# YuvalNirkin/hyperseg

Hardware: AMD Instinct MI355X
Metric: frames/sec @ bs=1 HyperSeg-M 1024x512 (higher is better)
Workload: dtype f32 storage and accumulation; level-4 inverted residual products as 3-term f16 splits (f32-class: 1.3e-7 of sum|a||b|; exact_f32 beside it)

## Files before the change

hyperseg_amd/_hip.py:

```python
import ctypes as C
import os

import torch

_LIB_PATH = os.environ.get('HS_HIP_LIB') or os.path.join(os.path.dirname(os.path.abspath(__file__)), 'lib',
                                                         'libhyperseg_hip.so')

ACT_NONE, ACT_RELU, ACT_RELU6, ACT_SWISH = 0, 1, 2, 3
PAD_MODES = {'zeros': 0, 'reflect': 1, 'replicate': 2, 'circular': 3}
PREV_NONE, PREV_SAME, PREV_BILINEAR = 0, 1, 2

_STATUS = {-1: 'bad argument', -2: 'feature map does not tile into the weight grid (H % fh or W % fw != 0)',
           -3: 'unsupported shape', -4: 'tile does not fit the LDS'}


class HipLibraryError(RuntimeError):
    pass


class StageInputC(C.Structure):
    _fields_ = [('skip', C.c_void_p), ('prev', C.c_void_p),
                ('batch', C.c_int32), ('H', C.c_int32), ('W', C.c_int32),
                ('c_skip', C.c_int32), ('c_prev', C.c_int32),
                ('Hp', C.c_int32), ('Wp', C.c_int32),
# ... 112 lines not shown
        'hs_patch_conv_plain_fwd': ([i32, vp, vp, i64, i32, i32, i32, i32, i32, i32, i32, i32, i32, i32, i32, vp, vp], C.c_int),
        'hs_patch_conv_plain_bwd_in': ([i32, vp, vp, i64, i32, i32, i32, i32, i32, i32, i32, i32, i32, i32, i32, vp, vp], C.c_int),
        'hs_patch_conv_plain_bwd_w': ([i32, vp, vp, i32, i32, i32, i32, i32, i32, i32, i32, i32, i32, i32, vp, i64, vp], C.c_int),
        'hs_depthwise_conv_fwd': ([vp, i32, i32, i32, i32, vp, i32, i32, i32, i32, i32, i32, vp, vp, i32, vp, vp, vp, vp, vp], C.c_int),
        'hs_pointwise_conv_fwd': ([vp, i32, i32, i32, vp, i32, vp, vp, vp, i32, vp, vp, vp], C.c_int),
        'hs_affine_act_fwd': ([vp, i32, i32, i32, vp, vp, i32, vp, vp, vp], C.c_int),
        'hs_patch_conv_bn_fwd': ([i32, vp, vp, vp, vp, vp, vp, C.c_float, C.c_float, i32, vp, vp, vp, vp, i64, i32, i32, i32, i32, i32, i32, i32, vp, vp], C.c_int),
        'hs_patch_conv_bn_bwd_w': ([i32, vp, vp, vp, vp, vp, vp, i32, i32, i32, i32, i32, i32, i32, i32, vp, i64, vp], C.c_int),
        'hs_bootstrap_mean_of_batch_fwd': ([vp, i32, i32, i32, C.c_float, vp, vp, vp, vp], C.c_int),
        'hs_bootstrap_mean_of_batch_bwd': ([vp, i32, i32, vp, vp, vp, vp], C.c_int),
        'hs_adam_blocks': ([vp, i32], C.c_int64),
        'hs_adam_step': ([vp, vp, vp, vp, vp, i32, vp, C.c_float, C.c_double, C.c_double, C.c_float, C.c_float, i32, i32, vp, vp], C.c_int),
        'hs_adam_step_amp': ([vp, vp, vp, vp, vp, i32, vp, C.c_float, C.c_double, C.c_double, C.c_float, C.c_float, i32, i32, vp, vp, vp, vp], C.c_int),
        'hs_depthwise_pool_blocks': ([i32, i32], C.c_int),
        'hs_depthwise_conv_se_fwd': ([vp, i32, i32, i32, i32, vp, i32, i32, i32, i32, i32, i32, vp, vp, i32, vp, vp, vp, C.POINTER(SeTailC), vp], C.c_int),
        'hs_mbconv_expand_dw_se_fwd': ([vp, i32, i32, i32, i32, vp, i32, vp, vp, vp, i32, i32, i32, i32, i32, i32, vp, vp, vp, C.POINTER(SeTailC), vp], C.c_int),
        'hs_se_tail_workspace': ([i32, i32, i32, i32, i64], C.c_int64),
        'hs_se_tail_tails': ([i32, i32, i32, i64], C.c_int),
        'hs_mbconv_se_workgroups': ([i32, i32, i32, i32, i32, i32], C.c_int64),
        'hs_stem_conv_fwd': ([vp, i32, i32, i32, i32, vp, i32, i32, i32, i32, i32, vp, vp, vp, vp], C.c_int),
        'hs_mbconv_tiles': ([i32, i32, i32, i32], C.c_int),
        'hs_stem_dw_fwd': ([vp, i32, i32, i32, vp, i32, vp, vp, i32, i32, i32, i32, vp, i32, i32, i32, vp, vp, vp, vp, vp], C.c_int),
        'hs_mbconv_expand_dw_fwd': ([vp, i32, i32, i32, i32, vp, i32, vp, vp, vp, i32, i32, i32, i32, i32, i32, vp, vp, vp, vp, vp], C.c_int),
        'hs_se_gate_fwd': ([vp, i32, i32, i32, C.c_float, vp, vp, i32, vp, vp, vp, vp, vp, i32, vp, vp, vp], C.c_int),
        'hs_gemm_split_kp': ([i32], C.c_int),
        'hs_gemm_split_fwd': ([vp, vp, vp, vp, vp, i32, vp, vp, i32, i32, i32, i32, i32, vp], C.c_int),
        'hs_gemm_split_conv2x2_fwd': ([vp, vp, vp, vp, i32, vp, vp, i32, i32, i32, i32, i32, i32, vp], C.c_int),
        'hs_gemm_split_up2_fwd': ([vp, vp, vp, vp, i32, vp, i32, i32, i32, i32, i32, i32, vp], C.c_int),
        'hs_pooled_shift_fwd': ([vp, i32, C.c_float, vp, vp, vp, i32, i32, vp], C.c_int),
    }
    for name, (argtypes, restype) in sig.items():
        fn = getattr(lib, name)
        fn.argtypes, fn.restype = argtypes, restype
    if lib.hs_version() != 1:
        raise HipLibraryError(f'ABI mismatch: library reports version {lib.hs_version()}, binding expects 1')
    return lib


lib = _load()
EXPORTS = ['hs_version', 'hs_build_info', 'hs_signal2weights_fwd', 'hs_signal2weights_multi_fwd', 'hs_s2w_pack_floats', 'hs_s2w_pack_fwd', 'hs_bank_pack_fwd', 'hs_bn_fold_fwd',
           'hs_patch_conv_fwd', 'hs_patch_conv_s2w_fwd', 'hs_k1_chain_workspace', 'hs_k1_chain_fwd', 'hs_decoder_chain_workspace', 'hs_decoder_chain_fwd', 'hs_meta_conv_fwd', 'hs_meta_conv_bwd', 'hs_patch_conv_gen_fwd', 'hs_patch_ir_fwd', 'hs_patch_ir_v0_fwd', 'hs_patch_ir_v0_ws_fwd', 'hs_patch_ir_v0_workspace', 'hs_patch_ir_route', 'hs_ir_tile_map', 'hs_upsample_bilinear_fwd', 'hs_upsample_argmax_fwd',
           'hs_stage_input_fwd', 'hs_depthwise_conv_fwd', 'hs_depthwise_pool_blocks', 'hs_stem_conv_fwd', 'hs_stem_dw_fwd', 'hs_mbconv_tiles', 'hs_mbconv_expand_dw_fwd', 'hs_se_gate_fwd', 'hs_depthwise_conv_se_fwd', 'hs_mbconv_expand_dw_se_fwd', 'hs_se_tail_workspace', 'hs_se_tail_tails', 'hs_mbconv_se_workgroups', 'hs_pointwise_conv_fwd', 'hs_affine_act_fwd', 'hs_gemm_split_kp', 'hs_gemm_split_fwd', 'hs_gemm_split_conv2x2_fwd', 'hs_gemm_split_up2_fwd', 'hs_pooled_shift_fwd', 'hs_patch_conv_bwd_input',
           'hs_patch_conv_bwd_weight', 'hs_halo_tiles_fwd', 'hs_halo_tiles_bwd', 'hs_tile_interior_fwd', 'hs_tile_interior_bwd', 'hs_dw_tiles_fwd', 'hs_dw_tiles_bwd_in', 'hs_dw_tiles_bwd_w',
           'hs_s2w_train_fwd', 'hs_s2w_train_workspace', 'hs_s2w_train_bwd', 'hs_cross_entropy_fwd', 'hs_cross_entropy_bwd', 'hs_cross_entropy_typed_fwd', 'hs_cross_entropy_typed_bwd', 'hs_bootstrapped_ce_fwd', 'hs_bootstrapped_ce_bwd', 'hs_bootstrap_mean_workspace', 'hs_bootstrap_mean_fwd', 'hs_bootstrap_mean_bwd', 'hs_bootstrap_mean_batched_fwd', 'hs_bootstrap_mean_batched_bwd', 'hs_bn_train_workspace', 'hs_bn_train_stats_fwd', 'hs_dw_tiles_bn_fwd', 'hs_dw_tiles_bn_bwd_w', 'hs_patch_conv_bn_fwd', 'hs_patch_conv_bn_bwd_w', 'hs_adam_blocks', 'hs_adam_step', 'hs_bootstrap_mean_of_batch_fwd', 'hs_bootstrap_mean_of_batch_bwd', 'hs_upsample_bilinear_bwd', 'hs_upsample_bilinear_typed_bwd', 'hs_upsample_bilinear_bf16_fwd', 'hs_stage_input_typed_fwd', 'hs_bank_unpack_fwd', 'hs_bn_act_train_fwd',
           'hs_bn_act_train_bwd', 'hs_dw_tiles_bn_bwd_in_partials', 'hs_dw_tiles_bn_bwd_in', 'hs_bn_act_train_bwd_apply', 'hs_patch_conv_plain_fwd', 'hs_patch_conv_plain_bwd_in', 'hs_patch_conv_plain_bwd_w',
           'hs_upsample_bilinear_f16_fwd', 'hs_adam_step_amp']


def check(status, what):
    if status == 0:
        return
    if status < 0:
        raise HipLibraryError(f'{what}: {_STATUS.get(status, status)}')
    raise HipLibraryError(f'{what}: HIP launch failed with hipError_t {status}')


def dev_ptr(t, name='tensor', dtype=torch.float32):
    if t is None:
        return None
    if not isinstance(t, torch.Tensor):
        raise TypeError(f'{name} must be a torch.Tensor')
    if not t.is_cuda:
        raise HipLibraryError(f'{name} is on {t.device}: the HyperSeg decoder path runs on an MI355X only '
                              '(hyperseg_amd has no CPU fallback)')
    if t.dtype != dtype:
# ... 26 lines not shown
```

hyperseg_amd/build.py:

```python
import os
import shutil
import subprocess
import sys

PKG = os.path.dirname(os.path.abspath(__file__))
REPO = os.path.dirname(PKG)
CSRC = os.path.join(PKG, 'csrc')
LIB_DIR = os.path.join(PKG, 'lib')
LIB_PATH = os.path.join(LIB_DIR, 'libhyperseg_hip.so')
SOURCES = ['hs_weights.hip', 'hs_patch_conv.hip', 'hs_patch_conv_gen.hip', 'hs_patch_conv_k1m.hip', 'hs_k1_chain.hip', 'hs_meta_conv.hip', 'hs_patch_ir.hip', 'hs_patch_ir_fused.hip', 'hs_patch_irc.hip', 'hs_patch_ir_px.hip', 'hs_patch_ir_d2.hip', 'hs_encoder.hip', 'hs_mbconv.hip', 'hs_mbconv_lean.hip', 'hs_gemm_split.hip', 'hs_patch_conv_bwd.hip', 'hs_patch_conv_train.hip', 'hs_train_aux.hip', 'hs_s2w_train.hip']
HEADERS = [os.path.join(CSRC, 'hs_common.h'), os.path.join(CSRC, 'hs_ir_tiles.h'), os.path.join(CSRC, 'hs_ir_common.h'), os.path.join(CSRC, 'hs_s2w_blocked.h'), os.path.join(CSRC, 'hs_se_tail.h'), os.path.join(REPO, 'include', 'hyperseg_hip.h')]
FLAGS = ['--offload-arch=gfx950', '-O3', '-std=c++17', '-fPIC', '-ffp-contract=off', '-mllvm', '-amdgpu-kernarg-preload-count=16',
         '-Wall', '-Wno-unused-function', '-I', os.path.join(REPO, 'include'), '-I', CSRC]


def _hipcc():
    for cand in (os.environ.get('HIPCC'), shutil.which('hipcc'), '/opt/rocm/bin/hipcc'):
        if cand and os.path.exists(cand):
            return cand
    raise RuntimeError('hipcc not found (need ROCm >= 7.0 with gfx950 support)')


def needs_build():
    if not os.path.exists(LIB_PATH):
        return True
    t = os.path.getmtime(LIB_PATH)
    deps = [os.path.join(CSRC, s) for s in SOURCES] + HEADERS + [os.path.abspath(__file__)]
    return any(os.path.getmtime(d) > t for d in deps)


def build(force=False, verbose=False, extra_flags=(), sources=None, lib_path=None, obj_suffix=''):
    if sources is None and lib_path is None and not force and not needs_build():
        return LIB_PATH
    sources = list(sources or SOURCES)
# ... 28 lines not shown
```

hyperseg_amd/csrc/hs_gemm_split.hip:

```cpp
#include "hs_common.h"
#include <type_traits>

namespace hs {

using half8 = __attribute__((ext_vector_type(8))) _Float16;
using gs_f32x4 = __attribute__((ext_vector_type(4))) float;

__device__ __forceinline__ int gs_exp_of(float m) { return min(max(__float_as_int(m) >> 23, 27), 254); }
__device__ __forceinline__ float gs_scale_of(int eb) { return __int_as_float((268 - eb) << 23); }
__device__ __forceinline__ float gs_inv_scale_of(int eb) { return __int_as_float((eb - 14) << 23); }

struct GemmSplitArgs {
    const _Float16* __restrict__ wf;
    const float* __restrict__ w_inv;
    const float* __restrict__ gate; const float* __restrict__ x;
    const float* shift;
    const float* residual;
    float* y;
    int M, K, KST, N, act;
    int conv_wo;
    float* pool_partial;
    int up2_wo;
};

#ifndef HS_GS_NARROW_MAX_WG
#define HS_GS_NARROW_MAX_WG 128
#endif

#ifndef HS_GS_TALL_MIN_WG
#define HS_GS_TALL_MIN_WG 257
#endif

template <int KS, int NWV, bool FAST, int NS, int MT, int NCH, bool PATCH>
// ... 114 lines not shown
#pragma unroll
                for (int j = 0; j < 8; ++j) {
                    const float mk = (FAST || PATCH ? k0 : k0 + j) < a.K ? 1.0f : 0.0f;
                    float g = mk;
                    if constexpr (!PATCH) g = gb ? gv[c][s][j] * mk : mk;
                    xv[c][t][s][j] *= g;
                    mx = max(mx, __float_as_uint(xv[c][t][s][j]) & 0x7fffffffu);
                }
            }
            {
                auto r16 = __builtin_amdgcn_permlane16_swap(mx, mx, false, false);
                mx = max(r16[0], r16[1]);
                auto r32 = __builtin_amdgcn_permlane32_swap(mx, mx, false, false);
                mx = max(r32[0], r32[1]);
            }
            const int eb = gs_exp_of(__uint_as_float(mx));
            const float sc = gs_scale_of(eb);
            invb[t] = gs_inv_scale_of(eb);
#pragma unroll
            for (int s = 0; s < KS; ++s) {
                if constexpr (FAST || PATCH) {
                    unsigned hh[4], ll[4];
#pragma unroll
                    for (int j = 0; j < 4; ++j) {
                        asm("v_fma_mixlo_f16 %0, %2, %4, 0\n\t"
                            "v_fma_mixhi_f16 %0, %3, %4, 0\n\t"
                            "v_fma_mixlo_f16 %1, %2, %4, -%0 op_sel_hi:[0,0,1]\n\t"
                            "v_fma_mixhi_f16 %1, %3, %4, -%0 op_sel:[0,0,1] op_sel_hi:[0,0,1]"
                            : "=&v"(hh[j]), "=&v"(ll[j]) : "v"(xv[c][t][s][2 * j]), "v"(xv[c][t][s][2 * j + 1]), "v"(sc));
                    }
                    using gs_u32x4 = __attribute__((ext_vector_type(4))) unsigned;
                    bh[t][s] = __builtin_bit_cast(half8, gs_u32x4{hh[0], hh[1], hh[2], hh[3]});
                    bl[t][s] = __builtin_bit_cast(half8, gs_u32x4{ll[0], ll[1], ll[2], ll[3]});
                } else {
#pragma unroll
                    for (int j = 0; j < 8; ++j) {
                        const float v = xv[c][t][s][j] * sc;
                        const _Float16 hi = (_Float16)v;
                        bh[t][s][j] = hi;
                        bl[t][s][j] = (_Float16)(v - (float)hi);
                    }
                }
            }
        }
        if (c == 0) {
            load_a(1);
            if constexpr (LATE_TAIL) load_tail();
        }
        __builtin_amdgcn_sched_barrier(0);
#pragma unroll
        for (int mt = 0; mt < MT; ++mt) {
            const int q = c * MT + mt;
            gs_f32x4 acc[NS];
#pragma unroll
// ... 207 lines not shown
```

hyperseg_amd/functional.py:

```python
import ctypes as C
import functools
import os
import threading

import torch

from . import _hip
from ._hip import ACT_NONE, ACT_RELU, ACT_RELU6, PAD_MODES

BN_EPS_DEFAULT = 1e-5
S2W_TRAIN_MAX_LAYERS = 8
USE_SIDE_STREAM = os.environ.get('HS_SIDE_STREAM', '0') == '1'
PIPELINE_BANKS = os.environ.get('HS_SIDE_STREAM', '0') == '2'
COSCHEDULE_BANKS = os.environ.get('HS_COSCHEDULE_BANKS', '0') == '1'


def _round_up(n, m):
    return (n + m - 1) // m * m


def _device_of(a):
    if isinstance(a, torch.Tensor):
        return a.device
    if isinstance(a, (StageInput, BankRef, SignalRef)):
# ... 830 lines not shown
            d, gate, _ws = desc
            st = _hip.lib.hs_mbconv_expand_dw_se_fwd(_hip.dev_ptr(x, 'x'), b, cin, h, w, _hip.dev_ptr(w_expand, 'w_expand'), cmid,
                                                     _hip.dev_ptr(scale0, 'scale0'), _hip.dev_ptr(shift0, 'shift0'),
                                                     _hip.dev_ptr(w_dw, 'w_dw'), k, stride, pad_top, pad_left, ho, wo,
                                                     _hip.dev_ptr(scale1, 'scale1'), _hip.dev_ptr(shift1, 'shift1'), y.data_ptr(),
                                                     C.byref(d), _hip.stream_ptr())
            _hip.check(st, 'hs_mbconv_expand_dw_se_fwd')
            return y, gate, True
    partial = None
    if pool:
        partial = torch.empty(b * cmid, _hip.lib.hs_mbconv_tiles(k, stride, ho, wo), device=x.device, dtype=torch.float32)
    st = _hip.lib.hs_mbconv_expand_dw_fwd(_hip.dev_ptr(x, 'x'), b, cin, h, w, _hip.dev_ptr(w_expand, 'w_expand'), cmid,
                                          _hip.dev_ptr(scale0, 'scale0'), _hip.dev_ptr(shift0, 'shift0'),
                                          _hip.dev_ptr(w_dw, 'w_dw'), k, stride, pad_top, pad_left, ho, wo,
                                          _hip.dev_ptr(scale1, 'scale1'), _hip.dev_ptr(shift1, 'shift1'), y.data_ptr(),
                                          partial.data_ptr() if pool else None, _hip.stream_ptr())
    _hip.check(st, 'hs_mbconv_expand_dw_fwd')
    if se is not None and pool:
        return y, partial, False
    return (y, partial) if pool else y


@_on_operand_device
def pointwise_conv(x, weight, gate=None, scale=None, shift=None, act=0, residual=None):
    b, cin, h, w = x.shape
    cout = weight.shape[0]
    y = torch.empty(b, cout, h, w, device=x.device, dtype=torch.float32)
    opt = lambda t, n: _hip.dev_ptr(t, n) if t is not None else None
    st = _hip.lib.hs_pointwise_conv_fwd(_hip.dev_ptr(x, 'x'), b, cin, h * w, _hip.dev_ptr(weight, 'weight'), cout,
                                        opt(gate, 'gate'), opt(scale, 'scale'), opt(shift, 'shift'), int(act),
                                        opt(residual, 'residual'), y.data_ptr(), _hip.stream_ptr())
    _hip.check(st, 'hs_pointwise_conv_fwd')
    return y


@_on_operand_device
def affine_act_(x, scale, shift, act=0, residual=None):
    b, c, h, w = x.shape
    st = _hip.lib.hs_affine_act_fwd(_hip.dev_ptr(x, 'x'), b, c, h * w,
                                    _hip.dev_ptr(scale, 'scale') if scale is not None else None,
                                    _hip.dev_ptr(shift, 'shift'), int(act),
                                    _hip.dev_ptr(residual, 'residual') if residual is not None else None, x.data_ptr(),
                                    _hip.stream_ptr())
    _hip.check(st, 'hs_affine_act_fwd')
    return x

# ... 216 lines not shown
```

hyperseg_amd/utils/inference.py:

```python
import contextlib
import os

import torch
import torch.nn as nn


@torch.no_grad()
def _fold(conv, bn):
    scale = bn.weight / torch.sqrt(bn.running_var + bn.eps)
    shift = bn.bias - bn.running_mean * scale
    conv.weight.mul_(scale.view(-1, 1, 1, 1))
    if conv.bias is not None:
        conv.bias.mul_(scale).add_(shift)
    else:
        conv.bias = nn.Parameter(shift.clone())


def _fold_pairs(module, pairs):
    n = 0
    for conv_name, bn_name in pairs:
        conv, bn = getattr(module, conv_name, None), getattr(module, bn_name, None)
        if isinstance(conv, nn.Conv2d) and isinstance(bn, nn.BatchNorm2d) and not bn.training:
            _fold(conv, bn)
            setattr(module, bn_name, nn.Identity())
# ... 3 lines not shown

def _fold_sequential(seq):
    n = 0
    mods = list(seq)
    for i in range(len(mods) - 1):
        if isinstance(mods[i], nn.Conv2d) and isinstance(mods[i + 1], nn.BatchNorm2d) and not mods[i + 1].training:
            _fold(mods[i], mods[i + 1])
            seq[i + 1] = nn.Identity()
            n += 1
    return n


def _bn_affine(bn):
    with torch.no_grad():
        scale = bn.weight / torch.sqrt(bn.running_var + bn.eps)
        shift = bn.bias - bn.running_mean * scale
    return scale.detach().clone(), shift.detach().clone()


SPLIT_GEMM_MAX_K = int(os.environ.get('HS_SPLIT_GEMM_MAX_K', '1280'))
STEM_DW = os.environ.get('HS_STEM_DW', '1') != '0'
FUSE_EXPAND_MIN_PIXELS = int(os.environ.get('HS_FUSE_EXPAND_MIN_PIXELS', '2048'))
FUSE_EXPAND_MAX_CIN = int(os.environ.get('HS_FUSE_EXPAND_MAX_CIN', '40'))


LEAN_MFMA_MAX_CIN = int(os.environ.get('HS_LEAN_MFMA_MAX_CIN', '16'))
PW_MFMA_MAX_CIN = int(os.environ.get('HS_PW_MFMA_MAX_CIN', '96'))
PW_MFMA_MIN_PIXELS = int(os.environ.get('HS_PW_MFMA_MIN_PIXELS', '8192'))
GEMM_LT_MIN_PIXELS = int(os.environ.get('HS_GEMM_LT_MIN_PIXELS', '16384'))


@contextlib.contextmanager
def gemm_library(pixels, batch=1):
    want = os.environ.get('HS_BLAS') or ('cublaslt' if (pixels >= GEMM_LT_MIN_PIXELS or batch > 1) else 'cublas')
    prev = torch.backends.cuda.preferred_blas_library()
    torch.backends.cuda.preferred_blas_library(want)
    try:
        yield
    finally:
        torch.backends.cuda.preferred_blas_library(prev)


class FusedPointwise(nn.Module):

    def __init__(self, conv, bn, act=0):
        super().__init__()
# ... 111 lines not shown
            self.pad_w, self.pad_h = conv._pad[0] + conv._pad[1], conv._pad[2] + conv._pad[3]
        else:
            self.pad_t, self.pad_l = conv.padding
            self.pad_h, self.pad_w = 2 * conv.padding[0], 2 * conv.padding[1]
        self.skip = blk.stride == 1 and blk.in_f == blk.out_f
        self._exp_t = None
        self._red_w = None
        self.se_tail = True
        self._stem = None
        if in_offset is not None:
            assert self.expand is not None, 'a depthwise conv cannot consume an offset tensor (zero padding)'
            self.expand.absorb_input_offset(in_offset)
        with torch.no_grad():
            carried = self.project.shift.clone()
            if self.skip and in_offset is not None:
                carried += in_offset.to(carried.device)
            self.defer_shift = bool(defer_shift)
            self.out_offset = carried.clone() if defer_shift else None
            self.project.shift.copy_(torch.zeros_like(carried) if defer_shift else carried)

    def fuses_expand(self, x, ho, wo):
        return self.expand is not None and x.shape[1] <= FUSE_EXPAND_MAX_CIN and ho * wo >= FUSE_EXPAND_MIN_PIXELS

    def forward(self, inputs, blk):
        from .. import functional as HF
        pre = None
        if self._stem is not None and inputs.shape[1] == 3:
            stem = self._stem[0]
            img = inputs.contiguous()
            pre = HF.stem_dw(img, stem.w28, stem.scale, stem.shift, stem.pad_t, stem.pad_l, stem.out_size(img),
                             blk._depthwise_conv.weight, self.pad_t, self.pad_l, self.scale, self.shift, pool=True) if STEM_DW else None
            inputs = pre[0] if pre is not None else stem(img)
        x = inputs.contiguous()
        b, _, h, w = x.shape
        ho = (h + self.pad_h - self.k) // self.stride + 1
        wo = (w + self.pad_w - self.k) // self.stride + 1
        lean = True
        red, exp = blk._se_reduce, blk._se_expand
        if self._exp_t is None or self._exp_t.device != x.device:
            self._exp_t = exp.weight.detach().flatten(1).t().contiguous()
        if self._red_w is None or self._red_w.device != x.device:
            self._red_w = red.weight.detach().flatten(1)
        proj = self.project
        cmid = blk._depthwise_conv.weight.shape[0]
        lean_gemm = lean and (cmid > LEAN_MFMA_MAX_CIN if self.defer_shift else not proj.mfma_covers(cmid, ho * wo))
        folds = lean_gemm and not (proj.split_gemm and proj.split_weights(True, x.device) is not None)
        se = (self._red_w, red.bias, self._exp_t, exp.bias) if self.se_tail and not folds else None
        if pre is not None:
            out = (pre[0], pre[1], False) if se is not None else pre
        elif self.fuses_expand(x, ho, wo):
            out = HF.mbconv_expand_dw(x, self.expand.conv.weight, self.expand.scale, self.expand.shift,
                                      blk._depthwise_conv.weight, self.stride, self.pad_t, self.pad_l, (ho, wo),
                                      self.scale, self.shift, pool=True, se=se)
        else:
            in_scale = in_shift = None
            if self.expand is not None:
                if lean and not self.expand.uses_mfma(x):
                    in_scale, in_shift = self.expand.scale, self.expand.shift
                    x = self.expand.raw(x)
                else:
                    x = self.expand(x)
            out = HF.depthwise_conv_bn_act(x, blk._depthwise_conv.weight, self.stride, self.pad_t, self.pad_l,
                                           (ho, wo), self.scale, self.shift, act=3, pool=True,
                                           in_scale=in_scale, in_shift=in_shift, se=se)
        y, pooled, gated = out if se is not None else (out[0], out[1], False)

        def se_gate(**fold):
            if gated and not fold:
                return pooled
            return HF.se_gate(pooled, b, ho * wo, red.weight, red.bias, self._exp_t, exp.bias, **fold)
        skip = inputs.contiguous() if self.skip else None
        if lean_gemm:
            sw = proj.split_weights(True, y.device) if proj.split_gemm else None
            if sw is not None:
                gate = se_gate()
                if self.defer_shift:
# ... 319 lines not shown
```

include/hyperseg_hip.h:

```cpp
#ifndef HYPERSEG_HIP_H
#define HYPERSEG_HIP_H

#include <stdint.h>

#ifdef __cplusplus
extern "C" {
#endif

#define HS_ABI_VERSION 1

typedef enum {
    HS_OK = 0,
    HS_ERR_BAD_ARG = -1,
    HS_ERR_NOT_DIVISIBLE = -2,
    HS_ERR_UNSUPPORTED = -3,
    HS_ERR_LDS = -4
} hs_status;

typedef enum { HS_ACT_NONE = 0, HS_ACT_RELU = 1, HS_ACT_RELU6 = 2, HS_ACT_SWISH = 3 } hs_act;
typedef enum { HS_PAD_ZEROS = 0, HS_PAD_REFLECT = 1, HS_PAD_REPLICATE = 2, HS_PAD_CIRCULAR = 3 } hs_pad_mode;
typedef enum { HS_PREV_NONE = 0, HS_PREV_SAME = 1, HS_PREV_BILINEAR = 2 } hs_prev_mode;

typedef struct {
    const float* skip;
// ... 158 lines not shown
                             const float* w, int32_t k, int32_t stride, int32_t pad_t, int32_t pad_l,
                             int32_t Ho, int32_t Wo, const float* scale, const float* shift, int32_t act,
                             float* y, const float* in_scale, const float* in_shift, const hs_se_tail* se, void* stream);
int hs_se_gate_fwd(const float* partial, int32_t batch, int32_t channels, int32_t nblk, float inv_hw,
                   const float* w_reduce, const float* b_reduce, int32_t c_squeezed, const float* w_expand,
                   const float* b_expand, float* squeezed, float* gate, const float* w_proj, int32_t c_out,
                   const float* out_scale, float* w_scaled, void* stream);


int hs_stem_conv_fwd(const float* x, int32_t batch, int32_t c_in, int32_t H, int32_t W, const float* w, int32_t c_out,
                     int32_t pad_t, int32_t pad_l, int32_t Ho, int32_t Wo, const float* scale, const float* shift,
                     float* y, void* stream);

int hs_mbconv_tiles(int32_t k, int32_t stride, int32_t Ho, int32_t Wo);
int hs_stem_dw_fwd(const float* x, int32_t batch, int32_t H, int32_t W, const float* w_stem28, int32_t c_mid,
                   const float* scale0, const float* shift0, int32_t stem_pad_t, int32_t stem_pad_l, int32_t Hs, int32_t Ws,
                   const float* w_dw, int32_t k, int32_t pad_t, int32_t pad_l, const float* scale1, const float* shift1,
                   float* y, float* pool_partial, void* stream);
int hs_mbconv_expand_dw_fwd(const float* x, int32_t batch, int32_t c_in, int32_t H, int32_t W,
                            const float* w_expand, int32_t c_mid, const float* scale0, const float* shift0,
                            const float* w_dw, int32_t k, int32_t stride, int32_t pad_t, int32_t pad_l,
                            int32_t Ho, int32_t Wo, const float* scale1, const float* shift1, float* y,
                            float* pool_partial, void* stream);
int64_t hs_mbconv_se_workgroups(int32_t batch, int32_t c_mid, int32_t k, int32_t stride, int32_t Ho, int32_t Wo);
int hs_mbconv_expand_dw_se_fwd(const float* x, int32_t batch, int32_t c_in, int32_t H, int32_t W,
                               const float* w_expand, int32_t c_mid, const float* scale0, const float* shift0,
                               const float* w_dw, int32_t k, int32_t stride, int32_t pad_t, int32_t pad_l,
                               int32_t Ho, int32_t Wo, const float* scale1, const float* shift1, float* y,
                               const hs_se_tail* se, void* stream);

int hs_pointwise_conv_fwd(const float* x, int32_t batch, int32_t c_in, int32_t pixels, const float* w, int32_t c_out,
                          const float* gate, const float* scale, const float* shift, int32_t act, const float* residual,
                          float* y, void* stream);

int hs_affine_act_fwd(const float* x, int32_t batch, int32_t channels, int32_t pixels, const float* scale,
                      const float* shift, int32_t act, const float* residual, float* y, void* stream);

int hs_gemm_split_kp(int32_t c_in);
int hs_gemm_split_fwd(const void* w_frag, const float* w_inv, const float* gate, const float* x, const float* shift,
                      int32_t act, const float* residual, float* y, int32_t batch, int32_t c_out, int32_t c_in, int32_t kp,
                      int32_t pixels, void* stream);
int hs_gemm_split_conv2x2_fwd(const void* w_frag, const float* w_inv, const float* x, const float* shift, int32_t act, float* y,
                              float* pool_partial, int32_t batch, int32_t c_out, int32_t c_in, int32_t kp, int32_t Ho,
                              int32_t Wo, void* stream);
int hs_gemm_split_up2_fwd(const void* w_frag, const float* w_inv, const float* x, const float* shift, int32_t act, float* y,
                          int32_t batch, int32_t c_out, int32_t c_in, int32_t kp, int32_t Ho, int32_t Wo, void* stream);
// ... 112 lines not shown
```

Baseline: 1354.

## Fuse split-f16 MFMA expand conv with depthwise conv for late MBConv blocks

Adds a kernel for later MBConv blocks (wider inputs, up to 96 channels) that runs the 1x1 expand conv as a 3-term f16-split MFMA GEMM straight into an LDS band tile. It then applies BN+swish, runs the depthwise conv with BN+swish from LDS, and writes per-band pool partials for SE. This avoids writing and reading back the expanded activation in global memory and saves a launch. In exchange, each workgroup recomputes halo rows, LDS use limits occupancy, and only certain shape instantiations are supported; other shapes fall back to the old path.

```diff
diff --git a/hyperseg_amd/_hip.py b/hyperseg_amd/_hip.py
--- a/hyperseg_amd/_hip.py
+++ b/hyperseg_amd/_hip.py
@@ -158,6 +158,8 @@
         'hs_mbconv_tiles': ([i32, i32, i32, i32], C.c_int),
         'hs_stem_dw_fwd': ([vp, i32, i32, i32, vp, i32, vp, vp, i32, i32, i32, i32, vp, i32, i32, i32, vp, vp, vp, vp, vp], C.c_int),
         'hs_mbconv_expand_dw_fwd': ([vp, i32, i32, i32, i32, vp, i32, vp, vp, vp, i32, i32, i32, i32, i32, i32, vp, vp, vp, vp, vp], C.c_int),
+        'hs_mbconv_late_pool_blocks': ([i32, i32, i32, i32, i32, i32, i32, i32, i32, i32, i32], C.c_int),
+        'hs_mbconv_late_fwd': ([vp, i32, i32, i32, i32, vp, vp, i32, i32, vp, vp, vp, i32, i32, i32, i32, i32, i32, vp, vp, vp, vp, i32, i32, vp], C.c_int),
         'hs_se_gate_fwd': ([vp, i32, i32, i32, C.c_float, vp, vp, i32, vp, vp, vp, vp, vp, i32, vp, vp, vp], C.c_int),
         'hs_gemm_split_kp': ([i32], C.c_int),
         'hs_gemm_split_fwd': ([vp, vp, vp, vp, vp, i32, vp, vp, i32, i32, i32, i32, i32, vp], C.c_int),
@@ -176,7 +178,7 @@
 lib = _load()
 EXPORTS = ['hs_version', 'hs_build_info', 'hs_signal2weights_fwd', 'hs_signal2weights_multi_fwd', 'hs_s2w_pack_floats', 'hs_s2w_pack_fwd', 'hs_bank_pack_fwd', 'hs_bn_fold_fwd',
            'hs_patch_conv_fwd', 'hs_patch_conv_s2w_fwd', 'hs_k1_chain_workspace', 'hs_k1_chain_fwd', 'hs_decoder_chain_workspace', 'hs_decoder_chain_fwd', 'hs_meta_conv_fwd', 'hs_meta_conv_bwd', 'hs_patch_conv_gen_fwd', 'hs_patch_ir_fwd', 'hs_patch_ir_v0_fwd', 'hs_patch_ir_v0_ws_fwd', 'hs_patch_ir_v0_workspace', 'hs_patch_ir_route', 'hs_ir_tile_map', 'hs_upsample_bilinear_fwd', 'hs_upsample_argmax_fwd',
-           'hs_stage_input_fwd', 'hs_depthwise_conv_fwd', 'hs_depthwise_pool_blocks', 'hs_stem_conv_fwd', 'hs_stem_dw_fwd', 'hs_mbconv_tiles', 'hs_mbconv_expand_dw_fwd', 'hs_se_gate_fwd', 'hs_depthwise_conv_se_fwd', 'hs_mbconv_expand_dw_se_fwd', 'hs_se_tail_workspace', 'hs_se_tail_tails', 'hs_mbconv_se_workgroups', 'hs_pointwise_conv_fwd', 'hs_affine_act_fwd', 'hs_gemm_split_kp', 'hs_gemm_split_fwd', 'hs_gemm_split_conv2x2_fwd', 'hs_gemm_split_up2_fwd', 'hs_pooled_shift_fwd', 'hs_patch_conv_bwd_input',
+           'hs_stage_input_fwd', 'hs_depthwise_conv_fwd', 'hs_depthwise_pool_blocks', 'hs_stem_conv_fwd', 'hs_stem_dw_fwd', 'hs_mbconv_tiles', 'hs_mbconv_expand_dw_fwd', 'hs_mbconv_late_pool_blocks', 'hs_mbconv_late_fwd', 'hs_se_gate_fwd', 'hs_depthwise_conv_se_fwd', 'hs_mbconv_expand_dw_se_fwd', 'hs_se_tail_workspace', 'hs_se_tail_tails', 'hs_mbconv_se_workgroups', 'hs_pointwise_conv_fwd', 'hs_affine_act_fwd', 'hs_gemm_split_kp', 'hs_gemm_split_fwd', 'hs_gemm_split_conv2x2_fwd', 'hs_gemm_split_up2_fwd', 'hs_pooled_shift_fwd', 'hs_patch_conv_bwd_input',
            'hs_patch_conv_bwd_weight', 'hs_halo_tiles_fwd', 'hs_halo_tiles_bwd', 'hs_tile_interior_fwd', 'hs_tile_interior_bwd', 'hs_dw_tiles_fwd', 'hs_dw_tiles_bwd_in', 'hs_dw_tiles_bwd_w',
            'hs_s2w_train_fwd', 'hs_s2w_train_workspace', 'hs_s2w_train_bwd', 'hs_cross_entropy_fwd', 'hs_cross_entropy_bwd', 'hs_cross_entropy_typed_fwd', 'hs_cross_entropy_typed_bwd', 'hs_bootstrapped_ce_fwd', 'hs_bootstrapped_ce_bwd', 'hs_bootstrap_mean_workspace', 'hs_bootstrap_mean_fwd', 'hs_bootstrap_mean_bwd', 'hs_bootstrap_mean_batched_fwd', 'hs_bootstrap_mean_batched_bwd', 'hs_bn_train_workspace', 'hs_bn_train_stats_fwd', 'hs_dw_tiles_bn_fwd', 'hs_dw_tiles_bn_bwd_w', 'hs_patch_conv_bn_fwd', 'hs_patch_conv_bn_bwd_w', 'hs_adam_blocks', 'hs_adam_step', 'hs_bootstrap_mean_of_batch_fwd', 'hs_bootstrap_mean_of_batch_bwd', 'hs_upsample_bilinear_bwd', 'hs_upsample_bilinear_typed_bwd', 'hs_upsample_bilinear_bf16_fwd', 'hs_stage_input_typed_fwd', 'hs_bank_unpack_fwd', 'hs_bn_act_train_fwd',
            'hs_bn_act_train_bwd', 'hs_dw_tiles_bn_bwd_in_partials', 'hs_dw_tiles_bn_bwd_in', 'hs_bn_act_train_bwd_apply', 'hs_patch_conv_plain_fwd', 'hs_patch_conv_plain_bwd_in', 'hs_patch_conv_plain_bwd_w',
diff --git a/hyperseg_amd/build.py b/hyperseg_amd/build.py
--- a/hyperseg_amd/build.py
+++ b/hyperseg_amd/build.py
@@ -8,8 +8,8 @@
 CSRC = os.path.join(PKG, 'csrc')
 LIB_DIR = os.path.join(PKG, 'lib')
 LIB_PATH = os.path.join(LIB_DIR, 'libhyperseg_hip.so')
-SOURCES = ['hs_weights.hip', 'hs_patch_conv.hip', 'hs_patch_conv_gen.hip', 'hs_patch_conv_k1m.hip', 'hs_k1_chain.hip', 'hs_meta_conv.hip', 'hs_patch_ir.hip', 'hs_patch_ir_fused.hip', 'hs_patch_irc.hip', 'hs_patch_ir_px.hip', 'hs_patch_ir_d2.hip', 'hs_encoder.hip', 'hs_mbconv.hip', 'hs_mbconv_lean.hip', 'hs_gemm_split.hip', 'hs_patch_conv_bwd.hip', 'hs_patch_conv_train.hip', 'hs_train_aux.hip', 'hs_s2w_train.hip']
-HEADERS = [os.path.join(CSRC, 'hs_common.h'), os.path.join(CSRC, 'hs_ir_tiles.h'), os.path.join(CSRC, 'hs_ir_common.h'), os.path.join(CSRC, 'hs_s2w_blocked.h'), os.path.join(CSRC, 'hs_se_tail.h'), os.path.join(REPO, 'include', 'hyperseg_hip.h')]
+SOURCES = ['hs_weights.hip', 'hs_patch_conv.hip', 'hs_patch_conv_gen.hip', 'hs_patch_conv_k1m.hip', 'hs_k1_chain.hip', 'hs_meta_conv.hip', 'hs_patch_ir.hip', 'hs_patch_ir_fused.hip', 'hs_patch_irc.hip', 'hs_patch_ir_px.hip', 'hs_patch_ir_d2.hip', 'hs_encoder.hip', 'hs_mbconv.hip', 'hs_mbconv_lean.hip', 'hs_gemm_split.hip', 'hs_mbconv_late.hip', 'hs_patch_conv_bwd.hip', 'hs_patch_conv_train.hip', 'hs_train_aux.hip', 'hs_s2w_train.hip']
+HEADERS = [os.path.join(CSRC, 'hs_common.h'), os.path.join(CSRC, 'hs_ir_tiles.h'), os.path.join(CSRC, 'hs_ir_common.h'), os.path.join(CSRC, 'hs_s2w_blocked.h'), os.path.join(CSRC, 'hs_se_tail.h'), os.path.join(CSRC, 'hs_gemm_split.h'),os.path.join(REPO, 'include', 'hyperseg_hip.h')]
 FLAGS = ['--offload-arch=gfx950', '-O3', '-std=c++17', '-fPIC', '-ffp-contract=off', '-mllvm', '-amdgpu-kernarg-preload-count=16',
          '-Wall', '-Wno-unused-function', '-I', os.path.join(REPO, 'include'), '-I', CSRC]
 
diff --git a/hyperseg_amd/csrc/hs_gemm_split.h b/hyperseg_amd/csrc/hs_gemm_split.h
--- /dev/null
+++ b/hyperseg_amd/csrc/hs_gemm_split.h
@@ -0,0 +1,22 @@
+#pragma once
+#include "hs_common.h"
+
+namespace hs {
+
+using half8 = __attribute__((ext_vector_type(8))) _Float16;
+using gs_f32x4 = __attribute__((ext_vector_type(4))) float;
+using gs_u32x4 = __attribute__((ext_vector_type(4))) unsigned;
+
+__device__ __forceinline__ int gs_exp_of(float m) { return min(max(__float_as_int(m) >> 23, 27), 254); }
+__device__ __forceinline__ float gs_scale_of(int eb) { return __int_as_float((268 - eb) << 23); }
+__device__ __forceinline__ float gs_inv_scale_of(int eb) { return __int_as_float((eb - 14) << 23); }
+
+__device__ __forceinline__ void gs_split2(float x0, float x1, float sc, unsigned& hh, unsigned& ll) {
+    asm("v_fma_mixlo_f16 %0, %2, %4, 0\n\t"
+        "v_fma_mixhi_f16 %0, %3, %4, 0\n\t"
+        "v_fma_mixlo_f16 %1, %2, %4, -%0 op_sel_hi:[0,0,1]\n\t"
+        "v_fma_mixhi_f16 %1, %3, %4, -%0 op_sel:[0,0,1] op_sel_hi:[0,0,1]"
+        : "=&v"(hh), "=&v"(ll) : "v"(x0), "v"(x1), "v"(sc));
+}
+
+}
diff --git a/hyperseg_amd/csrc/hs_gemm_split.hip b/hyperseg_amd/csrc/hs_gemm_split.hip
--- a/hyperseg_amd/csrc/hs_gemm_split.hip
+++ b/hyperseg_amd/csrc/hs_gemm_split.hip
@@ -1,14 +1,8 @@
 #include "hs_common.h"
+#include "hs_gemm_split.h"
 #include <type_traits>
 
 namespace hs {
-
-using half8 = __attribute__((ext_vector_type(8))) _Float16;
-using gs_f32x4 = __attribute__((ext_vector_type(4))) float;
-
-__device__ __forceinline__ int gs_exp_of(float m) { return min(max(__float_as_int(m) >> 23, 27), 254); }
-__device__ __forceinline__ float gs_scale_of(int eb) { return __int_as_float((268 - eb) << 23); }
-__device__ __forceinline__ float gs_inv_scale_of(int eb) { return __int_as_float((eb - 14) << 23); }
 
 struct GemmSplitArgs {
     const _Float16* __restrict__ wf;
@@ -169,14 +163,7 @@
                 if constexpr (FAST || PATCH) {
                     unsigned hh[4], ll[4];
 #pragma unroll
-                    for (int j = 0; j < 4; ++j) {
-                        asm("v_fma_mixlo_f16 %0, %2, %4, 0\n\t"
-                            "v_fma_mixhi_f16 %0, %3, %4, 0\n\t"
-                            "v_fma_mixlo_f16 %1, %2, %4, -%0 op_sel_hi:[0,0,1]\n\t"
-                            "v_fma_mixhi_f16 %1, %3, %4, -%0 op_sel:[0,0,1] op_sel_hi:[0,0,1]"
-                            : "=&v"(hh[j]), "=&v"(ll[j]) : "v"(xv[c][t][s][2 * j]), "v"(xv[c][t][s][2 * j + 1]), "v"(sc));
-                    }
-                    using gs_u32x4 = __attribute__((ext_vector_type(4))) unsigned;
+                    for (int j = 0; j < 4; ++j) gs_split2(xv[c][t][s][2 * j], xv[c][t][s][2 * j + 1], sc, hh[j], ll[j]);
                     bh[t][s] = __builtin_bit_cast(half8, gs_u32x4{hh[0], hh[1], hh[2], hh[3]});
                     bl[t][s] = __builtin_bit_cast(half8, gs_u32x4{ll[0], ll[1], ll[2], ll[3]});
                 } else {
diff --git a/hyperseg_amd/csrc/hs_mbconv_late.hip b/hyperseg_amd/csrc/hs_mbconv_late.hip
--- /dev/null
+++ b/hyperseg_amd/csrc/hs_mbconv_late.hip
@@ -0,0 +1,250 @@
+#include "hs_common.h"
+#include "hs_gemm_split.h"
+
+namespace hs {
+
+struct MlArgs {
+    const float* __restrict__ x;
+    const _Float16* __restrict__ wf;
+    const float* __restrict__ w_inv;
+    const float* __restrict__ s0; const float* __restrict__ b0;
+    const float* __restrict__ w_dw;
+    const float* __restrict__ s1; const float* __restrict__ b1;
+    float* __restrict__ y; float* __restrict__ pool;
+    int Cin, Cmid, KST, H, W, Ho, Wo, pad_t, pad_l, R, rows_in, tw;
+};
+
+template <int NK, int NS, int MT, int K, int S>
+__global__ __launch_bounds__(256)
+void mbconv_late_kernel(MlArgs a) {
+    extern __shared__ __attribute__((aligned(16))) float ml_tile[];
+    constexpr int G = 16 * MT, NP = 16 * NS, TPC = 256 / G;
+    const int tid = threadIdx.x, lane = tid & 63, wave = tid >> 6;
+    const int lrow = lane & 15, kg = lane >> 4;
+    const int band = blockIdx.x, b = blockIdx.z, c0 = blockIdx.y * G;
+    const int HW = a.H * a.W, rt_max = (a.Cmid + 15) >> 4;
+    const int yin0 = band * a.R * S - a.pad_t;
+    const int r_lo = max(0, -yin0), r_hi = min(a.rows_in, a.H - yin0);
+    const float* __restrict__ xb = a.x + (size_t)b * a.Cin * HW;
+
+    half8 ah[MT][NK], al[MT][NK];
+#pragma unroll
+    for (int mt = 0; mt < MT; ++mt) {
+        const int rt = min(blockIdx.y * MT + mt, rt_max - 1);
+#pragma unroll
+        for (int s = 0; s < NK; ++s) {
+            const _Float16* blk = a.wf + ((size_t)(rt * a.KST + s) * 2) * 512 + lane * 8;
+            ah[mt][s] = *reinterpret_cast<const half8*>(blk);
+            al[mt][s] = *reinterpret_cast<const half8*>(blk + 512);
+        }
+    }
+    float wi[MT][4], sc0[MT][4], sh0[MT][4];
+#pragma unroll
+    for (int mt = 0; mt < MT; ++mt)
+#pragma unroll
+        for (int r = 0; r < 4; ++r) {
+            const int ch = min(c0 + 16 * mt + 4 * kg + r, a.Cmid - 1);
+            wi[mt][r] = a.w_inv[ch]; sc0[mt][r] = a.s0[ch]; sh0[mt][r] = a.b0[ch];
+        }
+
+    for (int row = tid; row < G * a.rows_in; row += 256) {
+        float* tr = ml_tile + (size_t)row * a.tw;
+        const int r = row % a.rows_in;
+        if (r < r_lo || r >= r_hi) {
+            for (int t = 0; t < a.tw; t += 4) *reinterpret_cast<float4*>(tr + t) = make_float4(0.f, 0.f, 0.f, 0.f);
+        } else {
+            for (int t = 0; t < a.pad_l; ++t) tr[t] = 0.0f;
+            for (int t = a.pad_l + a.W; t < a.tw; ++t) tr[t] = 0.0f;
+        }
+    }
+
+    const int p_begin = (yin0 + r_lo) * a.W, p_end = (yin0 + r_hi) * a.W;
+    const int nblocks = r_hi > r_lo ? (p_end - p_begin + NP - 1) / NP : 0;
+    for (int pb = wave; pb < nblocks; pb += 4) {
+        const int p0 = p_begin + pb * NP;
+        const int pl = min(p0 + NS * lrow, p_end - NS);
+        float xv[NS][NK][8];
+#pragma unroll
+        for (int s = 0; s < NK; ++s)
+#pragma unroll
+            for (int j = 0; j < 8; ++j) {
+                const int kc = min(32 * s + 8 * kg + j, a.Cin - 1);
+                if constexpr (NS == 2) {
+                    const float2 v = *reinterpret_cast<const float2*>(xb + (size_t)kc * HW + pl);
+                    xv[0][s][j] = v.x; xv[1][s][j] = v.y;
+                } else {
+                    xv[0][s][j] = xb[(size_t)kc * HW + pl];
+                }
+            }
+        half8 bh[NS][NK], bl[NS][NK];
+        float invb[NS];
+#pragma unroll
+        for (int t = 0; t < NS; ++t) {
+            unsigned mx = 0;
+#pragma unroll
+            for (int s = 0; s < NK; ++s)
+#pragma unroll
+                for (int j = 0; j < 8; ++j) {
+                    xv[t][s][j] *= (32 * s + 8 * kg + j) < a.Cin ? 1.0f : 0.0f;
+                    mx = max(mx, __float_as_uint(xv[t][s][j]) & 0x7fffffffu);
+                }
+            {
+                auto r16 = __builtin_amdgcn_permlane16_swap(mx, mx, false, false);
+                mx = max(r16[0], r16[1]);
+                auto r32 = __builtin_amdgcn_permlane32_swap(mx, mx, false, false);
+                mx = max(r32[0], r32[1]);
+            }
+            const int eb = gs_exp_of(__uint_as_float(mx));
+            const float sc = gs_scale_of(eb);
+            invb[t] = gs_inv_scale_of(eb);
+#pragma unroll
+            for (int s = 0; s < NK; ++s) {
+                unsigned hh[4], ll[4];
+#pragma unroll
+                for (int j = 0; j < 4; ++j) gs_split2(xv[t][s][2 * j], xv[t][s][2 * j + 1], sc, hh[j], ll[j]);
+                bh[t][s] = __builtin_bit_cast(half8, gs_u32x4{hh[0], hh[1], hh[2], hh[3]});
+                bl[t][s] = __builtin_bit_cast(half8, gs_u32x4{ll[0], ll[1], ll[2], ll[3]});
+            }
+        }
+        int toff[NS];
+        bool live[NS];
+#pragma unroll
+        for (int t = 0; t < NS; ++t) {
+            const int p = p0 + NS * lrow + t;
+            live[t] = p < p_end;
+            const int yi = p / a.W, xi = p - yi * a.W;
+            toff[t] = (yi - yin0) * a.tw + a.pad_l + xi;
+        }
+#pragma unroll
+        for (int mt = 0; mt < MT; ++mt) {
+#pragma unroll
+            for (int t = 0; t < NS; ++t) {
+                gs_f32x4 acc = {0.f, 0.f, 0.f, 0.f};
+#pragma unroll
+                for (int s = 0; s < NK; ++s) {
+                    acc = __builtin_amdgcn_mfma_f32_16x16x32_f16(al[mt][s], bh[t][s], acc, 0, 0, 0);
+                    acc = __builtin_amdgcn_mfma_f32_16x16x32_f16(ah[mt][s], bl[t][s], acc, 0, 0, 0);
+                    acc = __builtin_amdgcn_mfma_f32_16x16x32_f16(ah[mt][s], bh[t][s], acc, 0, 0, 0);
+                }
+                if (live[t]) {
+#pragma unroll
+                    for (int r = 0; r < 4; ++r) {
+                        const float e = (acc[r] * invb[t]) * wi[mt][r];
+                        ml_tile[(size_t)(16 * mt + 4 * kg + r) * a.rows_in * a.tw + toff[t]] = swishf(fmaf(e, sc0[mt][r], sh0[mt][r]));
+                    }
+                }
+            }
+        }
+    }
+    __syncthreads();
+
+    const int g = tid / TPC, j0 = tid - g * TPC, c = c0 + g;
+    const int wq = a.Wo >> 2, rows_b = min(a.R, a.Ho - band * a.R);
+    float psum = 0.0f;
+    if (c < a.Cmid) {
+        float kd[K * K];
+#pragma unroll
+        for (int i = 0; i < K * K; ++i) kd[i] = a.w_dw[(size_t)c * K * K + i];
+        const float sc1 = a.s1[c], sh1 = a.b1[c];
+        constexpr int NCOL = 3 * S + K, NV = (NCOL + 3) / 4;
+        const float* gt = ml_tile + (size_t)g * a.rows_in * a.tw;
+        float* __restrict__ yc = a.y + ((size_t)b * a.Cmid + c) * a.Ho * a.Wo;
+        for (int q = j0; q < rows_b * wq; q += TPC) {
+            const int yo = q / wq, xo = (q - yo * wq) * 4;
+            float acc[4] = {0.f, 0.f, 0.f, 0.f};
+#pragma unroll
+            for (int ky = 0; ky < K; ++ky) {
+                const float* row = gt + (yo * S + ky) * a.tw + xo * S;
+                float v[NV * 4];
+#pragma unroll
+                for (int i = 0; i < NV; ++i) {
+                    const float4 t4 = *reinterpret_cast<const float4*>(row + 4 * i);
+                    v[4 * i] = t4.x; v[4 * i + 1] = t4.y; v[4 * i + 2] = t4.z; v[4 * i + 3] = t4.w;
+                }
+#pragma unroll
+                for (int kx = 0; kx < K; ++kx)
+#pragma unroll
+                    for (int t = 0; t < 4; ++t) acc[t] = fmaf(kd[ky * K + kx], v[t * S + kx], acc[t]);
+            }
+            float o[4];
+#pragma unroll
+            for (int t = 0; t < 4; ++t) o[t] = swishf(fmaf(acc[t], sc1, sh1));
+            *reinterpret_cast<float4*>(yc + (size_t)(band * a.R + yo) * a.Wo + xo) = make_float4(o[0], o[1], o[2], o[3]);
+            psum += (o[0] + o[1]) + (o[2] + o[3]);
+        }
+    }
+    if (a.pool) {
+#pragma unroll
+        for (int m = TPC / 2; m >= 1; m >>= 1) psum += __shfl_xor(psum, m, 64);
+        if (j0 == 0 && c < a.Cmid) a.pool[((size_t)b * a.Cmid + c) * gridDim.x + band] = psum;
+    }
+}
+
+static bool mbconv_late_plan(int c_in, int c_mid, int k, int stride, int Ho, int Wo, int& G, int& R) {
+    (void)Ho; (void)Wo;
+    const int nk = (c_in + 31) / 32;
+    const bool g32 = (nk == 3 && k == 3) || nk == 6 || (nk == 4 && stride == 2);
+    if (G <= 0) G = g32 && c_mid % 32 == 0 ? 32 : 16;
+    if (R <= 0) R = (nk == 3 && k == 3) || stride == 2 ? 2 : 4;
+    return (G == 16 || G == 32 || G == 64) && nk * (G / 16) <= 12 && (nk < 10 || G == 16);
+}
+
+}
+
+using namespace hs;
+
+static int mbconv_late_geometry(int32_t c_in, int32_t c_mid, int32_t k, int32_t stride, int32_t H, int32_t W, int32_t Ho, int32_t Wo,
+                                int32_t pad_l, int& G, int& R, int& rows_in, int& tw) {
+    if (c_in <= 0 || c_mid <= 0 || H <= 0 || W <= 0 || Ho <= 0 || Wo <= 0 || pad_l < 0) return HS_ERR_BAD_ARG;
+    if ((k != 3 && k != 5) || (stride != 1 && stride != 2) || (c_mid & 15) || (W & 1) || (Wo & 3)) return HS_ERR_UNSUPPORTED;
+    const int nk = (c_in + 31) / 32;
+    const bool inst = (nk == 3 && stride == 1) || (nk == 4 && k == 5) || (nk == 6 && stride == 1) || (nk == 10 && k == 3 && stride == 1);
+    if (!inst) return HS_ERR_UNSUPPORTED;
+    const bool auto_r = R <= 0, auto_g = G <= 0;
+    if (!mbconv_late_plan(c_in, c_mid, k, stride, Ho, Wo, G, R) || R < 1 || R > Ho) return HS_ERR_UNSUPPORTED;
+    tw = ((Wo - 1) * stride + k + 3) & ~3;
+    if (pad_l + W > tw) return HS_ERR_BAD_ARG;
+    auto lds = [&]() { return (size_t)G * ((R - 1) * stride + k) * tw * sizeof(float); };
+    while (auto_r && R > 1 && lds() > 64 * 1024) R = (R + 1) / 2;
+    if (auto_g && G > 16 && lds() > 64 * 1024) G = 16;
+    rows_in = (R - 1) * stride + k;
+    if (lds() > 64 * 1024) return HS_ERR_UNSUPPORTED;
+    return HS_OK;
+}
+
+extern "C" int hs_mbconv_late_pool_blocks(int32_t c_in, int32_t c_mid, int32_t k, int32_t stride, int32_t H, int32_t W,
+                                          int32_t Ho, int32_t Wo, int32_t pad_l, int32_t group, int32_t band_rows) {
+    int G = group, R = band_rows, rows_in, tw;
+    const int st = mbconv_late_geometry(c_in, c_mid, k, stride, H, W, Ho, Wo, pad_l, G, R, rows_in, tw);
+    return st != HS_OK ? st : (Ho + R - 1) / R;
+}
+
+extern "C" int hs_mbconv_late_fwd(const float* x, int32_t batch, int32_t c_in, int32_t H, int32_t W, const void* w_frag,
+                                  const float* w_inv, int32_t kp, int32_t c_mid, const float* scale0, const float* shift0,
+                                  const float* w_dw, int32_t k, int32_t stride, int32_t pad_t, int32_t pad_l, int32_t Ho, int32_t Wo,
+                                  const float* scale1, const float* shift1, float* y, float* pool_partial, int32_t group,
+                                  int32_t band_rows, void* stream) {
+    if (!x || !w_frag || !w_inv || !scale0 || !shift0 || !w_dw || !scale1 || !shift1 || !y || batch <= 0 || pad_t < 0) return HS_ERR_BAD_ARG;
+    int G = group, R = band_rows, rows_in, tw;
+    const int st = mbconv_late_geometry(c_in, c_mid, k, stride, H, W, Ho, Wo, pad_l, G, R, rows_in, tw);
+    if (st != HS_OK) return st;
+    if (kp < 32 * ((c_in + 31) / 32) || (kp & 31)) return HS_ERR_BAD_ARG;
+    if ((((size_t)x) & 7) != 0 || (((size_t)y) & 15) != 0 || batch > 65535) return HS_ERR_UNSUPPORTED;
+    MlArgs a{x, (const _Float16*)w_frag, w_inv, scale0, shift0, w_dw, scale1, shift1, y, pool_partial,
+             c_in, c_mid, kp / 32, H, W, Ho, Wo, pad_t, pad_l, R, rows_in, tw};
+    dim3 grid((Ho + R - 1) / R, (c_mid + G - 1) / G, batch);
+    const size_t lds = (size_t)G * rows_in * tw * sizeof(float);
+    hipStream_t s = (hipStream_t)stream;
+    const int nk = (c_in + 31) / 32, mt = G / 16;
+#define HS_ML(NK, NS, MT, KK, SS) hipLaunchKernelGGL((mbconv_late_kernel<NK, NS, MT, KK, SS>), grid, dim3(256), lds, s, a)
+#define HS_ML_MT2(NK, KK, SS) do { if (mt == 1) HS_ML(NK, 2, 1, KK, SS); else HS_ML(NK, 2, 2, KK, SS); } while (0)
+#define HS_ML_MT4(NK, KK, SS) do { if (mt == 4) HS_ML(NK, 2, 4, KK, SS); else HS_ML_MT2(NK, KK, SS); } while (0)
+    if (nk == 3) { if (k == 3) HS_ML_MT4(3, 3, 1); else HS_ML_MT4(3, 5, 1); }
+    else if (nk == 4) { if (stride == 1) HS_ML_MT2(4, 5, 1); else HS_ML_MT2(4, 5, 2); }
+    else if (nk == 6) { if (k == 3) HS_ML_MT2(6, 3, 1); else HS_ML_MT2(6, 5, 1); }
+    else HS_ML(10, 1, 1, 3, 1);
+#undef HS_ML_MT4
+#undef HS_ML_MT2
+#undef HS_ML
+    return launch_status();
+}
diff --git a/hyperseg_amd/functional.py b/hyperseg_amd/functional.py
--- a/hyperseg_amd/functional.py
+++ b/hyperseg_amd/functional.py
@@ -876,6 +876,30 @@
 
 
 @_on_operand_device
+def mbconv_late(x, sw, scale0, shift0, w_dw, stride, pad_top, pad_left, out_size, scale1, shift1, group=0, band_rows=0):
+    b, cin, h, w = x.shape
+    if cin != sw.c_in:
+        raise ValueError(f'input has {cin} channels, the weight {sw.c_in}')
+    cmid, k = w_dw.shape[0], w_dw.shape[-1]
+    ho, wo = out_size
+    nblk = _hip.lib.hs_mbconv_late_pool_blocks(cin, cmid, k, stride, h, w, ho, wo, pad_left, group, band_rows)
+    if nblk == -3:
+        return None
+    _hip.check(min(nblk, 0), 'hs_mbconv_late_pool_blocks')
+    y = torch.empty(b, cmid, ho, wo, device=x.device, dtype=torch.float32)
+    partial = torch.empty(b * cmid, nblk, device=x.device, dtype=torch.float32)
+    st = _hip.lib.hs_mbconv_late_fwd(_hip.dev_ptr(x, 'x'), b, cin, h, w, _hip.dev_ptr(sw.frag, 'w_frag', torch.float16),
+                                     _hip.dev_ptr(sw.inv, 'w_inv'), sw.kp, cmid, _hip.dev_ptr(scale0, 'scale0'),
+                                     _hip.dev_ptr(shift0, 'shift0'), _hip.dev_ptr(w_dw, 'w_dw'), k, stride, pad_top, pad_left, ho, wo,
+                                     _hip.dev_ptr(scale1, 'scale1'), _hip.dev_ptr(shift1, 'shift1'), y.data_ptr(), partial.data_ptr(),
+                                     group, band_rows, _hip.stream_ptr())
+    if st == -3:
+        return None
+    _hip.check(st, 'hs_mbconv_late_fwd')
+    return y, partial
+
+
+@_on_operand_device
 def pointwise_conv(x, weight, gate=None, scale=None, shift=None, act=0, residual=None):
     b, cin, h, w = x.shape
     cout = weight.shape[0]
diff --git a/hyperseg_amd/utils/inference.py b/hyperseg_amd/utils/inference.py
--- a/hyperseg_amd/utils/inference.py
+++ b/hyperseg_amd/utils/inference.py
@@ -49,6 +49,7 @@
 STEM_DW = os.environ.get('HS_STEM_DW', '1') != '0'
 FUSE_EXPAND_MIN_PIXELS = int(os.environ.get('HS_FUSE_EXPAND_MIN_PIXELS', '2048'))
 FUSE_EXPAND_MAX_CIN = int(os.environ.get('HS_FUSE_EXPAND_MAX_CIN', '40'))
+LATE_FUSE_MAX_CIN = int(os.environ.get('HS_LATE_FUSE_MAX_CIN', '96'))
 
 
 LEAN_MFMA_MAX_CIN = int(os.environ.get('HS_LEAN_MFMA_MAX_CIN', '16'))
@@ -206,6 +207,17 @@
     def fuses_expand(self, x, ho, wo):
         return self.expand is not None and x.shape[1] <= FUSE_EXPAND_MAX_CIN and ho * wo >= FUSE_EXPAND_MIN_PIXELS
 
+    def _late(self, x, blk, ho, wo):
+        from .. import functional as HF
+        exp = self.expand
+        if HF.SE_TAIL or exp is None or not exp.split_gemm or not x.is_cuda or x.shape[0] != 1 or x.shape[1] > LATE_FUSE_MAX_CIN or exp.uses_mfma(x):
+            return None
+        sw = exp.split_weights(False, x.device)
+        if sw is None:
+            return None
+        return HF.mbconv_late(x, sw, exp.scale, exp.shift, blk._depthwise_conv.weight, self.stride, self.pad_t, self.pad_l, (ho, wo),
+                              self.scale, self.shift)
+
     def forward(self, inputs, blk):
         from .. import functional as HF
         pre = None
@@ -236,6 +248,8 @@
             out = HF.mbconv_expand_dw(x, self.expand.conv.weight, self.expand.scale, self.expand.shift,
                                       blk._depthwise_conv.weight, self.stride, self.pad_t, self.pad_l, (ho, wo),
                                       self.scale, self.shift, pool=True, se=se)
+        elif (late := self._late(x, blk, ho, wo)) is not None:
+            out = (late[0], late[1], False) if se is not None else late
         else:
             in_scale = in_shift = None
             if self.expand is not None:
diff --git a/include/hyperseg_hip.h b/include/hyperseg_hip.h
--- a/include/hyperseg_hip.h
+++ b/include/hyperseg_hip.h
@@ -204,6 +204,12 @@
                             const float* w_dw, int32_t k, int32_t stride, int32_t pad_t, int32_t pad_l,
                             int32_t Ho, int32_t Wo, const float* scale1, const float* shift1, float* y,
                             float* pool_partial, void* stream);
+int hs_mbconv_late_pool_blocks(int32_t c_in, int32_t c_mid, int32_t k, int32_t stride, int32_t H, int32_t W, int32_t Ho, int32_t Wo,
+                               int32_t pad_l, int32_t group, int32_t band_rows);
+int hs_mbconv_late_fwd(const float* x, int32_t batch, int32_t c_in, int32_t H, int32_t W, const void* w_frag, const float* w_inv,
+                       int32_t kp, int32_t c_mid, const float* scale0, const float* shift0, const float* w_dw, int32_t k,
+                       int32_t stride, int32_t pad_t, int32_t pad_l, int32_t Ho, int32_t Wo, const float* scale1,
+                       const float* shift1, float* y, float* pool_partial, int32_t group, int32_t band_rows, void* stream);
 int64_t hs_mbconv_se_workgroups(int32_t batch, int32_t c_mid, int32_t k, int32_t stride, int32_t Ho, int32_t Wo);
 int hs_mbconv_expand_dw_se_fwd(const float* x, int32_t batch, int32_t c_in, int32_t H, int32_t W,
                                const float* w_expand, int32_t c_mid, const float* scale0, const float* shift0,
```

Result: no change. 1366 (median of 6 runs) (+0.9%).
